# lijx10/SO-Net

Measured on AMD Instinct MI355X. Metric: point-clouds/sec forward, ModelNet40 5k-pt 8x8 SOM, higher is better.
Workload: dtype f32 (operands split into fp16 pieces, 3 fp16 MFMAs per product, f32 accumulate; parity 1e-5)

## Files before the change

include/sonet_hip.h:

```cpp
#ifndef SONET_HIP_H
#define SONET_HIP_H

#include <stddef.h>
#include <stdint.h>

#ifdef __cplusplus
extern "C" {
#endif

typedef void *sonet_stream_t;

enum {
    SONET_OK = 0,
    SONET_ERR_INVALID_ARG = 1,
    SONET_ERR_UNSUPPORTED = 2,
    SONET_ERR_LAUNCH = 3,
    SONET_ERR_NO_DEVICE = 4
};

int sonet_abi_version(void);
const char *sonet_build_arch(void);
const char *sonet_last_error(void);
int sonet_check_device(void);
int sonet_diag_mfma_f16_rate(int random_operands, int iters, double *tflops_out, double *ghz_out, sonet_stream_t stream);
// ... 208 lines not shown
                                  int B, int C, int L, sonet_stream_t stream);
int sonet_node_add_affine_act_f32(float *t, const float *z, const int32_t *min_idx_i32, const float *scale,
                                  const float *shift, int relu, int B, int C, int L, int M, sonet_stream_t stream);

size_t sonet_pointmlp_stats_ws_size(int B, int Cout, int L);
int sonet_pointmlp_h3_stats_f32(const float *x1, int C1, const float *x2, int C2, const void *Wp3, const float *scale,
                                const float *shift, int relu, float *y, int B, int Cout, int L, void *stats_ws,
                                float *mean, float *var, sonet_stream_t stream);
int sonet_pointmlp_x3_stats_f32(const float *x1, int C1, const float *x2, int C2, const void *Wp3, const float *scale,
                                const float *shift, int relu, float *y, int B, int Cout, int L, void *stats_ws,
                                float *mean, float *var, sonet_stream_t stream);

int sonet_pointmlp_h3_nodeadd_f32(const float *x1, int C1, const float *x2, int C2, const void *Wp3, const float *scale,
                                  const float *shift, int relu, float *y, int B, int Cout, int L,
                                  const float *zadd, const int32_t *zidx, int ZM, sonet_stream_t stream);
int sonet_pointmlp_h3_nodeadd_stats_f32(const float *x1, int C1, const float *x2, int C2, const void *Wp3, const float *scale,
                                        const float *shift, int relu, float *y, int B, int Cout, int L,
                                        const float *zadd, const int32_t *zidx, int ZM, void *stats_ws,
                                        float *mean, float *var, sonet_stream_t stream);

size_t sonet_pointmlp_bf16_stats_ws_size(int B, int Cout, int L);
int sonet_pointmlp_bf16_stats(const uint16_t *x1, int C1, const uint16_t *x2, int C2, const void *Wp,
                              const float *scale, const float *shift, int relu, uint16_t *y,
                              int B, int Cout, int L, void *stats_ws, float *mean, float *var, sonet_stream_t stream);
int sonet_pointmlp_bf16_pool(const uint16_t *x1, int C1, const uint16_t *x2, int C2, const void *Wp,
                             const float *scale, const float *shift, int relu, const int32_t *ids, const int32_t *row_max,
                             int32_t *out_idx, float *out_val, int B, int Cout, int L, int M, sonet_stream_t stream);
int sonet_pointmlp_bf16_stats_xaff(const uint16_t *x1, int C1, const uint16_t *x2, int C2, const void *Wp,
                                   const float *scale, const float *shift, int relu, uint16_t *y,
                                   int B, int Cout, int L, void *stats_ws, float *mean, float *var,
                                   const float *xs1, const float *xh1, const float *xs2, const float *xh2, int xrelu,
                                   sonet_stream_t stream);
int sonet_pointmlp_bf16_pool_xaff(const uint16_t *x1, int C1, const uint16_t *x2, int C2, const void *Wp,
                                  const float *scale, const float *shift, int relu, const int32_t *ids, const int32_t *row_max,
                                  int32_t *out_idx, float *out_val, int B, int Cout, int L, int M,
                                  const float *xs1, const float *xh1, const float *xs2, const float *xh2, int xrelu,
                                  sonet_stream_t stream);

size_t sonet_pointmlp_h3_segpool_ws_size(int B, int Cout, int M);
int sonet_pointmlp_h3_segpool_f32(const float *x1, int C1, const float *x2, int C2, const void *Wp3, const float *scale,
                                  const float *shift, int relu, const int32_t *ids_sorted, const int32_t *pos0,
                                  const int32_t *row_max, int M, void *ws, int32_t *out_idx, float *out_val,
                                  int B, int Cout, int L, const float *xs1, const float *xh1, const float *xs2, const float *xh2,
                                  int xrelu, sonet_stream_t stream);
int sonet_pointmlp_h3_stats_xaff_f32(const float *x1, int C1, const float *x2, int C2, const void *Wp3, const float *scale,
                                     const float *shift, int relu, float *y, int B, int Cout, int L, void *stats_ws,
                                     float *mean, float *var, const float *xs1, const float *xh1, const float *xs2, const float *xh2,
                                     int xrelu, sonet_stream_t stream);

size_t sonet_wgrad_x3_ws_size(int B, int Cout, int Cin, int L);
int sonet_wgrad_x3_f32(const float *g, const float *x, float *dw, void *ws, int B, int Cout, int Cin, int L, sonet_stream_t stream);
int sonet_wgrad_x3_xaff_f32(const float *g, const float *x, float *dw, void *ws, int B, int Cout, int Cin, int L,
                            const float *xs, const float *xh, int xrelu, sonet_stream_t stream);
size_t sonet_wgrad_bf16_ws_size(int B, int Cout, int Cin, int L);
int sonet_wgrad_bf16(const uint16_t *g, const uint16_t *x, float *dw, void *ws, int B, int Cout, int Cin, int L, sonet_stream_t stream);
int sonet_wgrad_bf16_xaff(const uint16_t *g, const uint16_t *x, float *dw, void *ws, int B, int Cout, int Cin, int L,
                          const float *xs, const float *xh, int xrelu, sonet_stream_t stream);
int sonet_node_gather_lead_affine_act_f32(const float *z, const int32_t *gidx, const float *lead, const float *wl,
                                          const float *scale, const float *shift, int relu, float *out,
                                          int B, int C, int L, int M, int NL, sonet_stream_t stream);

int sonet_node_gather_lead_affine_act_bf16(const uint16_t *z, const int32_t *gidx, const float *lead, const float *wl,
                                           const float *scale, const float *shift, int relu, uint16_t *out,
                                           int B, int C, int L, int M, int NL, sonet_stream_t stream);

int sonet_linear_act_f32(const float *x, const float *W, const float *scale, const float *shift, int relu, float *y,
                         int B, int Cin, int Cout, sonet_stream_t stream);

size_t sonet_pooled_dgrad_ws_size(int B, int C, int M, int L);
int sonet_pooled_wgrad_f32(const float *g_pooled, const int32_t *pos, const float *x, int B, int C, int M, int Ci, int L,
                           float *gw_partial, sonet_stream_t stream);
int sonet_pooled_wgrad_xaff_f32(const float *g_pooled, const int32_t *pos, const float *x, int B, int C, int M, int Ci, int L,
                                float *gw_partial, const float *xs, const float *xh, int xrelu, sonet_stream_t stream);
int sonet_pooled_dgrad_f32(const float *g_pooled, const int32_t *pos, const float *W, int B, int C, int M, int C1, int C2,
                           int L, void *ws, float *gx1, float *gx2, sonet_stream_t stream);
int sonet_pooled_wgrad_xbf16(const float *g_pooled, const int32_t *pos, const uint16_t *x, int B, int C, int M, int Ci, int L,
                             float *gw_partial, sonet_stream_t stream);
int sonet_pooled_wgrad_xaff_xbf16(const float *g_pooled, const int32_t *pos, const uint16_t *x, int B, int C, int M, int Ci, int L,
                                  float *gw_partial, const float *xs, const float *xh, int xrelu, sonet_stream_t stream);
int sonet_pooled_dgrad_obf16(const float *g_pooled, const int32_t *pos, const float *W, int B, int C, int M, int C1, int C2,
                             int L, void *ws, uint16_t *gx1, uint16_t *gx2, sonet_stream_t stream);
int sonet_pooled_dgrad_mfma_bf16(const float *g_pooled, const int32_t *pos, const void *wt_pack, int B, int C, int M, int C1, int C2,
                                 int L, void *ws, uint16_t *gx1, uint16_t *gx2, sonet_stream_t stream);

int sonet_bn_fwd_coeffs_f32(const float *mean, const float *var, const float *gamma, const float *beta, float eps, int C,
                            float *invstd, float *scale, float *shift, sonet_stream_t stream);
int sonet_bn_running_update_f32(float *running_mean, float *running_var, const float *mean, const float *var,
                                float momentum, float unbias, int C, sonet_stream_t stream);
int sonet_bn_rider_set(const float *gamma, const float *beta, float eps, float momentum, float unbias,
                       float *running_mean, float *running_var, float *invstd, float *scale, float *shift);
int sonet_bn_bwd_coeffs_f32(const double *sums, const float *mean, const float *invstd, const float *gamma, double n, int C,
                            float *a, float *b, float *c0, float *g_gamma, float *g_beta, sonet_stream_t stream);
int sonet_chunk_mean_f32(const float *h, float *out, long long rows, int N, int k, sonet_stream_t stream);
int sonet_channel_affine_act_out_f32(const float *x, const float *scale, const float *shift, int relu, float *y,
                                     int B, int C, int L, sonet_stream_t stream);

int sonet_channel_stats_f32(const float *y, int B, int C, int L, double *stat_ws,
                            float *mean, float *var_biased, sonet_stream_t stream);
int sonet_channel_affine_act_f32(float *y, const float *scale, const float *shift, int relu,
                                 int B, int C, int L, sonet_stream_t stream);

int sonet_chamfer_nn_f32(const float *q, const float *db, int32_t *nn, int B, int Nq, int Nd,
                         sonet_stream_t stream);
size_t sonet_chamfer_loss_ws_size(int B, int M, int N);
int sonet_chamfer_loss_f32(const float *pred, const float *gt, int32_t *nn_pg , int32_t *nn_gp ,
                           float *elem_fwd , float *elem_bwd , double *sums, void *ws, int B, int M,
                           int N, sonet_stream_t stream);
int sonet_chamfer_grad_f32(const float *pred, const float *gt, const int32_t *nn_pg, const int32_t *nn_gp, const float *elem_fwd,
                           const float *elem_bwd, const float *gscale, float *dpred, int32_t *bad, int B, int M, int N,
                           sonet_stream_t stream);
size_t sonet_seg_metrics_ws_size(int B, int C, int N);
int sonet_seg_metrics_f32(const float *score, const int64_t *seg, const int64_t *label, const int32_t *part_offsets, int n_cat,
                          int32_t *pred_out , int32_t *correct, double *nll_sum, int32_t *inter, int32_t *pred_cnt,
                          int32_t *gt_cnt, double *iou, int32_t *bad, void *ws, int B, int C, int N, sonet_stream_t stream);
int sonet_retrieval_chunk_keys(void);
size_t sonet_retrieval_ws_size(int N, int D, int Q, int top);
int sonet_retrieval_lists_f32(const float *feat, const int64_t *label , const int64_t *ids ,
                              const int32_t *query , int n_label, int top, int64_t *nn_id, float *nn_dist,
                              int32_t *nn_pos , int32_t *count, int32_t *label_out , int32_t *bad,
                              void *ws, int N, int D, int Q, sonet_stream_t stream);
#define SONET_UPCONV_TILE_PIXELS 128
#define SONET_UPCONV_K_CHUNK 16
#define SONET_UPCONV_COUT_BLOCK 32
#define SONET_UPCONV_MAX_HW 64
size_t sonet_upconv3x3_pack_size(int Cin, int Cout);
int sonet_upconv3x3_pack_f32(const float *W, void *Wp, int Cin, int Cout, sonet_stream_t stream);
int sonet_upconv3x3_f32(const float *x, const void *Wp, const float *scale, const float *shift, int relu, float *y,
                        int B, int Cin, int Cout, int H, int W, uint32_t *range_log, sonet_stream_t stream);
size_t sonet_upconv3x3_dgrad_pack_size(int Cin, int Cout);
int sonet_upconv3x3_dgrad_pack_f32(const float *W, void *Wpt, int Cin, int Cout, sonet_stream_t stream);
int sonet_upconv3x3_dgrad_f32(const float *g, const void *Wpt, float *dx, int B, int Cin, int Cout, int H, int W, sonet_stream_t stream);
#define SONET_UPWGRAD_K_STEP 16
#define SONET_UPWGRAD_CIN_BLOCK 32
#define SONET_UPWGRAD_FLUSH_COLS 256
#define SONET_UPWGRAD_SLICE_COLS 512
#define SONET_UPWGRAD_MAX_SLICES 128
size_t sonet_upconv3x3_wgrad_ws_size(int B, int Cin, int Cout, int H, int W);
int sonet_upconv3x3_wgrad_f32(const float *g, const float *x, float *dw, void *ws, int B, int Cin, int Cout, int H, int W,
                              sonet_stream_t stream);
#ifdef SONET_VARIANTS
int sonet_pointmlp_h3_kmax_f32(const float *x1, int C1, const float *x2, int C2, const void *Wp3, const float *scale,
                               const float *shift, int relu, float *out, void *keys_ws, int B, int Cout, int L, int M,
                               sonet_stream_t stream);

size_t sonet_chamfer_nn2_ws_size(int B, int Na, int Nb);
int sonet_chamfer_nn2_f32(const float *a, const float *b, int32_t *nn_ab, int32_t *nn_ba, void *ws, int B, int Na, int Nb,
                          sonet_stream_t stream);

size_t sonet_pooled_dgrad_tail_ws_size(int B, int C2, int L);
int sonet_pooled_dgrad_tail_f32(const float *g_pooled, const int32_t *pos, const float *W, int B, int C, int M, int C1, int C2,
                                int L, void *ws, float *gx1, float *gx2, const float *col0, const int32_t *pos0,
                                const float *sraw, const float *ssc, const float *ssh, int srelu, void *tail_ws, double *sums,
                                sonet_stream_t stream);
#endif

int sonet_pointmlp_x3_pack_strided(const float *W, long long row_stride, long long col_stride, void *Wp3, int Cin, int Cout, int rows,
                                   sonet_stream_t stream);
int sonet_pointmlp_h3_pack_strided(const float *W, long long row_stride, long long col_stride, void *Wp3, int Cin, int Cout, int rows,
                                   sonet_stream_t stream);
int sonet_pack_multi(const void *table, int n_entries, int total_blocks, sonet_stream_t stream);
int sonet_pack_multi_kc(int flavour, int Cin);
int sonet_pointmlp_bf16_pack_strided(const float *W, long long row_stride, long long col_stride, void *Wp, int Cin, int Cout, int rows,
                                     sonet_stream_t stream);

int sonet_adam_chunk(void);
int sonet_adam_multi_f32(const void *tensors, const float *step_size, const float *bc2_sqrt, const int32_t *chunk_tensor,
                         const long long *chunk_off, const long long *sizes, int nchunks, float beta1, float beta2,
                         float one_minus_beta1, float one_minus_beta2, float eps, sonet_stream_t stream);

int sonet_fc_max_rows(void);
int sonet_fc_bn_act_fwd_f32(const float *x, const float *W, const float *bias, const float *gamma, const float *beta,
                            float *running_mean, float *running_var, float momentum, float eps, int relu, int B, int Cin, int Cout,
                            float *y, float *xhat, float *invstd, sonet_stream_t stream);
int sonet_fc_bn_act_bwd_f32(const float *gy, const float *y, const float *xhat, const float *invstd, const float *gamma, const float *x,
                            int relu, int B, int Cin, int Cout, float *dz, float *dW, float *dbias, float *dgamma, float *dbeta,
                            sonet_stream_t stream);
int sonet_fc_dx_f32(const float *dz, const float *W, int B, int Cin, int Cout, float *dx, sonet_stream_t stream);

#ifdef __cplusplus
}
#endif
#endif
```

so-net_amd/csrc/knn_layer.hip:

```cpp
#include "common.hpp"
#include "knn_h1.hpp"

namespace {

constexpr int KL_STAGE = 8;
constexpr int KL_MAXC = 512;
constexpr int KL_WRING = 4;

struct KnnLayerArgs {
    const int4 *rec;
    const uint4 *zp;
    const float *wl, *scale1, *shift1;
    const uint4 *Wp;
    const float *scale2, *shift2;
    char *yp;
    unsigned *rlog;
    long long Lm;
    int relu1, relu2, KC, NS, KCP, CT, Cout, GK, G, ngout, Lout;
    int abl;
};

struct KnnLayerLds {
    uint4 x[2][KL_STAGE][2][2][128];
    float coef[5][KL_MAXC];
    float aff[KL_MAXC / 32][2][2][16];
    unsigned wmax[4];
};
static_assert(sizeof(KnnLayerLds) <= 160 * 1024, "LDS of a CU");
static_assert(4 * 32 * GM_STRIDE * sizeof(float) <= sizeof(uint4) * 2 * KL_STAGE * 2 * 2 * 128, "the epilogue's staging fits the operand buffers");

template <int MT>
__global__ __launch_bounds__(256) void knn_layer2_gmax_kernel(const KnnLayerArgs a)
{
    __shared__ __attribute__((aligned(16))) KnnLayerLds lds;
    const int tid = (int)threadIdx.x;
    const int lane = tid & 63, wave = __builtin_amdgcn_readfirstlane(tid >> 6);
    const int j = lane & 31, h = lane >> 5;
    const int blk = (int)blockIdx.x;
    const int col = tid & 127, hh = __builtin_amdgcn_readfirstlane(tid >> 7);
    const int4 rcol = a.rec[(long long)blk * 128 + col];
    const KnnCol kcol = knn_col(rcol);
    const int KC = a.KC, Cin = KC * 16;

    for (int t = tid; t < KL_MAXC; t += 256) {
        const int c = (t >> 4) * 16 + p16_channel((t >> 3) & 1, t & 7);
#pragma unroll
        for (int kind = 0; kind < 5; ++kind) lds.coef[kind][t] = knn_h1_coef(kind, c < Cin, c, a.wl, a.scale1, a.shift1);
    }
    for (int o = tid; o < a.Cout; o += 256) {
        const int rr = o & 31;
        float *t = &lds.aff[o >> 5][(rr >> 2) & 1][0][(rr & 3) | ((rr >> 3) << 2)];
        t[0] = a.scale2[o] * (32.f / 1024.f);
        t[16] = a.shift2[o] * 32.f;
    }

    RangeAcc xr = {0, 0u};
    const float lo1 = a.relu1 ? 0.f : -65504.f;
    const uint4 *zbase = a.zp + (long long)hh * a.Lm + (kcol.ok ? rcol.x : 0);

    uint4 Zh[2], Zm[2];
    unsigned hv4[4], mv4[4];
    f32x2_t creg[2][5];
    auto load_coef = [&](f32x2_t (&c)[5], int kc, int u) {
        const int ci = (kc < KC ? kc : KC - 1) * 16 + hh * 8 + 2 * u;
#pragma unroll
        for (int kind = 0; kind < 5; ++kind) c[kind] = *reinterpret_cast<const f32x2_t *>(&lds.coef[kind][ci]);
    };
    auto gather = [&](int slot, int kc) {
        kc = kc < KC ? kc : KC - 1;
        const uint4 *zq = zbase + (long long)kc * 4 * a.Lm;
#ifdef SONET_VARIANTS
        if (a.abl & 2) zq = a.zp + (long long)hh * a.Lm;
#endif
        Zh[slot] = zq[0];
        Zm[slot] = zq[2 * a.Lm];
    };
    auto build_unit = [&](int slot, const f32x2_t (&c)[5], int kc, int buf, int q, int u) {
        const bool in = kc < KC, live = kcol.ok && in;
        const float *const cf[5] = {reinterpret_cast<const float *>(&c[0]), reinterpret_cast<const float *>(&c[1]), reinterpret_cast<const float *>(&c[2]),
                                    reinterpret_cast<const float *>(&c[3]), reinterpret_cast<const float *>(&c[4])};
        KnnCol kk = kcol;
        kk.valid = kcol.valid && in;
        const unsigned zh = u == 0 ? Zh[slot].x : u == 1 ? Zh[slot].y : u == 2 ? Zh[slot].z : Zh[slot].w;
        const unsigned zm = u == 0 ? Zm[slot].x : u == 1 ? Zm[slot].y : u == 2 ? Zm[slot].z : Zm[slot].w;
        knn_h1_pair<false>(live ? zh : 0u, live ? zm : 0u, cf, kk, lo1, xr, hv4[u], mv4[u]);
        if (u == 3) {
            lds.x[buf][q][0][hh][col] = make_uint4(hv4[0], hv4[1], hv4[2], hv4[3]);
            lds.x[buf][q][1][hh][col] = make_uint4(mv4[0], mv4[1], mv4[2], mv4[3]);
        }
    };

    const int NS = a.NS, KCT = NS * KL_STAGE;
    const uint4 *wbase = a.Wp + ((size_t)(wave * MT) * a.KCP * 2) * 64 + lane;
    uint4 Wr[KL_WRING][2];
    auto load_w = [&](int kc0, int t) {
        int kc = kc0 + t / MT;
        kc = kc < KCT ? kc : KCT - 1;
        const uint4 *wq = wbase + ((size_t)(t % MT) * a.KCP + kc) * 128;
#ifdef SONET_VARIANTS
        if (a.abl & 1) wq = wbase;
#endif
        Wr[t % KL_WRING][0] = wq[0];
        Wr[t % KL_WRING][1] = wq[64];
    };

    f32x16 acc[MT][4];
#pragma unroll
    for (int mt = 0; mt < MT; ++mt)
#pragma unroll
        for (int c = 0; c < 4; ++c)
#pragma unroll
            for (int r = 0; r < 16; ++r) acc[mt][c][r] = 0.f;

    f16x8 Bf[2][2][4];
    auto read_b = [&](int set, int buf, int q) {
#pragma unroll
        for (int c = 0; c < 4; ++c) {
            Bf[set][0][c] = __builtin_bit_cast(f16x8, lds.x[buf][q][0][h][32 * c + j]);
            Bf[set][1][c] = __builtin_bit_cast(f16x8, lds.x[buf][q][1][h][32 * c + j]);
        }
    };

#pragma unroll
    for (int t = 0; t < KL_WRING - 1; ++t) load_w(0, t);
    {
        uint4 Ph[KL_STAGE], Pm[KL_STAGE];
#pragma unroll
        for (int q = 0; q < KL_STAGE; ++q) {
            gather(0, q);
            Ph[q] = Zh[0];
            Pm[q] = Zm[0];
        }
        __syncthreads();
#pragma unroll
        for (int q = 0; q < KL_STAGE; ++q) {
            Zh[0] = Ph[q];
            Zm[0] = Pm[q];
            f32x2_t c4[4][5];
#pragma unroll
            for (int u = 0; u < 4; ++u) load_coef(c4[u], q, u);
#pragma unroll
            for (int u = 0; u < 4; ++u) build_unit(0, c4[u], q, 0, q, u);
        }
    }
    if (NS > 1) load_coef(creg[0], KL_STAGE, 0);

    auto stage = [&](int s, auto build_next) {
        constexpr bool BUILD = decltype(build_next)::value;
        const int buf = s & 1, kc0 = s * KL_STAGE, kn = kc0 + KL_STAGE;
        __syncthreads();
        read_b(0, buf, 0);
        if constexpr (BUILD) gather(0, kn);
#pragma unroll
        for (int q = 0; q < KL_STAGE; ++q) {
#pragma unroll
            for (int mt = 0; mt < MT; ++mt) {
                const int t = q * MT + mt;
                load_w(kc0, t + KL_WRING - 1);
                if (mt == 0 && q + 1 < KL_STAGE) {
                    read_b((q + 1) & 1, buf, q + 1);
                    if constexpr (BUILD) gather((q + 1) & 1, kn + q + 1);
                }
                const f16x8 wh = __builtin_bit_cast(f16x8, Wr[t % KL_WRING][0]), wm = __builtin_bit_cast(f16x8, Wr[t % KL_WRING][1]);
#pragma unroll
                for (int term = 0; term < 3; ++term)
#pragma unroll
                    for (int c = 0; c < 4; ++c)
                        acc[mt][c] = __builtin_amdgcn_mfma_f32_32x32x16_f16(term == 0 ? wm : wh, Bf[q & 1][term == 1 ? 1 : 0][c], acc[mt][c], 0, 0, 0);
#pragma unroll
                for (int u = 0; u < 4; ++u)
                    if (BUILD && u * MT / 4 == mt) {
                        const int n = q * 4 + u;
                        load_coef(creg[(n + 1) & 1], kn + (n + 1) / 4, (n + 1) % 4);
                        build_unit(q & 1, creg[n & 1], kn + q, buf ^ 1, q, u);
                    }
#define KL_GAP2 __builtin_amdgcn_sched_group_barrier(0x008, 1, 0); __builtin_amdgcn_sched_group_barrier(0x002, 3, 0); \
                __builtin_amdgcn_sched_group_barrier(0x008, 1, 0); __builtin_amdgcn_sched_group_barrier(0x002, 4, 0);
                KL_GAP2 KL_GAP2 KL_GAP2 KL_GAP2 KL_GAP2 KL_GAP2
#undef KL_GAP2
                __builtin_amdgcn_sched_barrier(0);
            }
        }
    };
    for (int s = 0; s + 1 < NS; ++s) stage(s, bool_c<true>{});
    stage(NS - 1, bool_c<false>{});
    __syncthreads();

    float (*gm)[GM_STRIDE] = reinterpret_cast<float (*)[GM_STRIDE]>(reinterpret_cast<char *>(&lds.x[0][0][0][0][0]) + (size_t)wave * (32 * GM_STRIDE * 4));
    RangeAcc yr = {0, 0u};
    const float relu_thr = a.relu2 ? 0.f : -__builtin_inff();
    const float split_lo = a.relu2 ? 0.f : -2047.f;
    int tid2 = tid;
    asm volatile("" : "+v"(tid2));
    const int je = tid2 & 31, he = (tid2 >> 5) & 1;
    const int p = tid2 & 3, g = (tid2 & 63) >> 2;
    const long long n_out = (long long)blk * a.G + g;
    const bool node = g < a.G && n_out < a.ngout;
    const float *rbase = &gm[2 * (p & 1) + 8 * (p >> 1)][(g < a.G ? g : 0) * a.GK];
#pragma unroll
    for (int mt = 0; mt < MT; ++mt) {
        const int ct = wave * MT + mt;
        float sc16[16], sh16[16];
        {
            const float4 *t4 = reinterpret_cast<const float4 *>(&lds.aff[ct][he][0][0]);
#pragma unroll
            for (int u = 0; u < 4; ++u) {
                const float4 s4 = t4[u], h4 = t4[4 + u];
                sc16[4 * u] = s4.x; sc16[4 * u + 1] = s4.y; sc16[4 * u + 2] = s4.z; sc16[4 * u + 3] = s4.w;
                sh16[4 * u] = h4.x; sh16[4 * u + 1] = h4.y; sh16[4 * u + 2] = h4.z; sh16[4 * u + 3] = h4.w;
            }
        }
#pragma unroll
        for (int c = 0; c < 4; ++c)
#pragma unroll
            for (int r = 0; r < 16; ++r) {
                const float v = __fmaf_rn(acc[mt][c][r], sc16[r], sh16[r]);
                gm[(r & 3) + 8 * (r >> 2) + 4 * he][32 * c + je] = v < relu_thr ? 0.f : v;
            }
        __builtin_amdgcn_fence(__ATOMIC_RELEASE, "wavefront");
        __builtin_amdgcn_wave_barrier();
        __builtin_amdgcn_fence(__ATOMIC_ACQUIRE, "wavefront");
        float m0[4], m1[4];
#pragma unroll
        for (int qh = 0; qh < 4; ++qh) {
            const float *r0 = rbase + (16 * (qh >> 1) + 4 * (qh & 1)) * GM_STRIDE;
            m0[qh] = r0[0];
            m1[qh] = r0[GM_STRIDE];
        }
        for (int k = 1; k < a.GK; ++k) {
#pragma unroll
            for (int qh = 0; qh < 4; ++qh) {
                const float *r0 = rbase + (16 * (qh >> 1) + 4 * (qh & 1)) * GM_STRIDE;
                m0[qh] = nan_max(m0[qh], r0[k]);
                m1[qh] = nan_max(m1[qh], r0[GM_STRIDE + k]);
            }
        }
        if (node) {
#pragma unroll
            for (int qh = 0; qh < 4; ++qh) {
                const int qq = qh >> 1, h2 = qh & 1;
                gmax_p16_store(m0[qh], m1[qh], split_lo, yr, a.yp, ct * 2 + qq, h2, p, (size_t)a.Lout, (size_t)n_out);
            }
        }
        __builtin_amdgcn_fence(__ATOMIC_RELEASE, "wavefront");
        __builtin_amdgcn_wave_barrier();
        __builtin_amdgcn_fence(__ATOMIC_ACQUIRE, "wavefront");
    }

    if (a.rlog != nullptr) {
        const unsigned b1 = range_x32_out(wave_umax(range_act_bits(xr, a.relu1)));
        const unsigned b2 = range_x32_out(wave_umax(range_act_bits(yr, a.relu2)));
        if ((tid2 & 63) == 0) lds.wmax[wave] = b1 > b2 ? b1 : b2;
        __syncthreads();
        if (tid2 == 0) {
            const unsigned m01 = lds.wmax[0] > lds.wmax[1] ? lds.wmax[0] : lds.wmax[1], m23 = lds.wmax[2] > lds.wmax[3] ? lds.wmax[2] : lds.wmax[3];
            const unsigned mx = m01 > m23 ? m01 : m23;
            if (mx > __atomic_load_n(a.rlog + 2, __ATOMIC_RELAXED)) atomicMax(a.rlog + 2, mx);
            if (blk == 0) atomicMax(a.rlog + 1, reinterpret_cast<const unsigned *>(a.Wp + (size_t)a.CT * a.KCP * 128)[0]);
        }
    }
}

}

extern "C" int sonet_knn_layer2_gmax_p16(const void *rec, const void *z_p16, const float *wl, const float *scale1, const float *shift1, int relu1,
                                         int B, int M, int K, int Cin, const void *Wp, const float *scale2, const float *shift2, int relu2,
                                         int Cout, int GK, int G, int ngout, int Lout, void *yp, sonet_stream_t stream)
{
    const char *what = "sonet_knn_layer2_gmax_p16";
    SONET_REQUIRE(rec && z_p16 && wl && scale1 && shift1 && Wp && scale2 && shift2 && yp, "%s: NULL pointer", what);
    SONET_REQUIRE(B > 0 && M > 0 && Cin > 0 && Cout > 0 && K >= 1 && K <= 128, "%s: bad size B=%d M=%d Cin=%d Cout=%d K=%d", what, B, M, Cin, Cout, K);
    SONET_REQUIRE(GK == K && G == knn_stage_groups(K) && (long long)ngout == (long long)B * M, "%s: the grouping of the K-level layout is GK=%d G=%d ngout=%d", what,
                  K, knn_stage_groups(K), B * M);
    SONET_REQUIRE(Lout >= ngout, "%s: Lout=%d (the planes' column count) below ngout=%d", what, Lout, ngout);
    if (Cout % 128 != 0 || Cout > KL_MAXC) return sonet::fail(SONET_ERR_UNSUPPORTED, "%s: Cout=%d must be a multiple of 128, at most %d", what, Cout, KL_MAXC);
    if (Cin % 16 != 0 || Cin > KL_MAXC) return sonet::fail(SONET_ERR_UNSUPPORTED, "%s: Cin=%d must be a multiple of 16, at most %d", what, Cin, KL_MAXC);
    if (G * GK > 128) return sonet::fail(SONET_ERR_UNSUPPORTED, "%s: G GK = %d columns exceed a block", what, G * GK);
    const long long Lp = (long long)sonet_knn_stage_columns(B, M, K), Lm = (long long)sonet_node_stage_columns(B, M);
    const long long nblk = Lp / 128;
    const int KC = Cin / 16, NS = sonet::ceil_div(KC, KL_STAGE), KCP = NS * KL_STAGE, CT = Cout / 32;
    if (nblk > 0x7FFFFFFFll || (double)KC * 64.0 * (double)Lm >= 2.0e9 || (double)(Cout / 16) * 64.0 * (double)Lout >= 2.0e9 || (double)CT * KCP * 2048.0 >= 2.0e9)
        return sonet::fail(SONET_ERR_UNSUPPORTED, "%s: a panel exceeds 2 GiB", what);
    KnnLayerArgs a;
    a.rec = reinterpret_cast<const int4 *>(rec); a.zp = reinterpret_cast<const uint4 *>(z_p16); a.wl = wl; a.scale1 = scale1; a.shift1 = shift1;
    a.Wp = reinterpret_cast<const uint4 *>(Wp); a.scale2 = scale2; a.shift2 = shift2; a.yp = static_cast<char *>(yp); a.rlog = sonet::range_log();
    a.Lm = Lm; a.relu1 = relu1; a.relu2 = relu2; a.KC = KC; a.NS = NS; a.KCP = KCP; a.CT = CT; a.Cout = Cout; a.GK = GK; a.G = G; a.ngout = ngout; a.Lout = Lout;
    a.abl = 0;
#ifdef SONET_VARIANTS
    sonet::knob_int("SONET_KL_ABL", &a.abl);
#endif
    with_int_c<1, 2, 3, 4>(Cout / 128, [&](auto mt) {
        hipLaunchKernelGGL((knn_layer2_gmax_kernel<decltype(mt)::value>), dim3((unsigned)nblk), dim3(256), 0, sonet::as_stream(stream), a);
    });
    return sonet::launched(what);
}
```

so-net_amd/sonet_hip/_lib.py:

```python
import ctypes
import os

import torch

_HERE = os.path.dirname(os.path.abspath(__file__))
LIB_PATH = os.path.join(os.path.dirname(_HERE), "lib", "libsonet_hip.so")
VARIANTS_PATH = os.path.join(os.path.dirname(_HERE), "lib", "libsonet_hip_variants.so")
if os.environ.get("SONET_HIP_LIB"):
    LIB_PATH = os.environ["SONET_HIP_LIB"]

_vp = ctypes.c_void_p
_i = ctypes.c_int

SIGNATURES = {
    "sonet_abi_version": [],
    "sonet_build_arch": [],
    "sonet_last_error": [],
    "sonet_check_device": [],
    "sonet_range_log_set": [_vp],
    "sonet_pooled_wgrad_f32": [_vp, _vp, _vp, _i, _i, _i, _i, _i, _vp, _vp],
    "sonet_bn_running_update_f32": [_vp, _vp, _vp, _vp, ctypes.c_float, ctypes.c_float, _i, _vp],
    "sonet_knn_prepare_f32": [_vp, _vp, _i, _i, _i, _i, _vp, _vp, _vp, _vp],
    "sonet_pointmlp_h3_gather_f32": [_vp, _i, _i, _vp, _vp, _i, _vp, _vp, _vp, _i, _vp, _i, _i, _i, _vp],
    "sonet_planes_max_f32": [_vp, _vp, ctypes.c_longlong, _i, _i, _vp],
# ... 36 lines not shown
    "sonet_pointmlp_bf16_pack": [_vp, _vp, _i, _i, _vp],
    "sonet_pointmlp_bf16": [_vp, _i, _vp, _i, _vp, _vp, _vp, _i, _vp, _i, _i, _i, _vp],
    "sonet_pointmlp_bf16_acc": [_vp, _i, _vp, _i, _vp, _vp, _vp, _i, _vp, _vp, _i, _i, _i, _vp],
    "sonet_pointmlp_bf16_bnb": [_vp, _vp, _i, _vp, _vp, _vp, _vp, _vp, _vp, _vp, _vp, _i, _vp, _vp, _vp, _i, _i, _i, _vp],
    "sonet_pointmlp_bf16_gather": [_vp, _i, _i, _vp, _vp, _i, _vp, _vp, _vp, _i, _vp, _i, _i, _i, _vp],
    "sonet_index_max_gather_bf16": [_vp, _vp, _vp, _vp, _vp, _i, _i, _i, _i, _vp],
    "sonet_index_max_gather_p16": [_vp, _vp, _vp, _vp, _vp, _i, _i, _i, _i, _vp],
    "sonet_node_gather_lead_affine_act_f32": [_vp, _vp, _vp, _vp, _vp, _vp, _i, _vp, _i, _i, _i, _i, _i, _vp],
    "sonet_node_gather_lead_affine_act_bf16": [_vp, _vp, _vp, _vp, _vp, _vp, _i, _vp, _i, _i, _i, _i, _i, _vp],
    "sonet_pointmlp_stats_ws_size": [_i, _i, _i],
    "sonet_pointmlp_h3_stats_f32": [_vp, _i, _vp, _i, _vp, _vp, _vp, _i, _vp, _i, _i, _i, _vp, _vp, _vp, _vp],
    "sonet_pointmlp_x3_stats_f32": [_vp, _i, _vp, _i, _vp, _vp, _vp, _i, _vp, _i, _i, _i, _vp, _vp, _vp, _vp],
    "sonet_pointmlp_bf16_stats_ws_size": [_i, _i, _i],
    "sonet_pointmlp_bf16_stats": [_vp, _i, _vp, _i, _vp, _vp, _vp, _i, _vp, _i, _i, _i, _vp, _vp, _vp, _vp],
    "sonet_pointmlp_bf16_stats_xaff": [_vp, _i, _vp, _i, _vp, _vp, _vp, _i, _vp, _i, _i, _i, _vp, _vp, _vp, _vp, _vp, _vp, _vp, _i, _vp],
    "sonet_pointmlp_h3_nodeadd_f32": [_vp, _i, _vp, _i, _vp, _vp, _vp, _i, _vp, _i, _i, _i, _vp, _vp, _i, _vp],
    "sonet_pointmlp_h3_nodeadd_stats_f32": [_vp, _i, _vp, _i, _vp, _vp, _vp, _i, _vp, _i, _i, _i, _vp, _vp, _i, _vp, _vp, _vp, _vp],
    "sonet_wgrad_x3_ws_size": [_i, _i, _i, _i],
    "sonet_wgrad_x3_f32": [_vp, _vp, _vp, _vp, _i, _i, _i, _i, _vp],
    "sonet_wgrad_bf16_ws_size": [_i, _i, _i, _i],
    "sonet_wgrad_bf16": [_vp, _vp, _vp, _vp, _i, _i, _i, _i, _vp],
    "sonet_wgrad_bf16_xaff": [_vp, _vp, _vp, _vp, _i, _i, _i, _i, _vp, _vp, _i, _vp],
    "sonet_pointmlp_x3_pack_size": [_i, _i],
    "sonet_pointmlp_x3_pack": [_vp, _vp, _i, _i, _vp],
    "sonet_pointmlp_x3_f32": [_vp, _i, _vp, _i, _vp, _vp, _vp, _i, _vp, _i, _i, _i, _vp],
    "sonet_pointmlp_h3_pack": [_vp, _vp, _i, _i, _vp],
    "sonet_pointmlp_h3_f32": [_vp, _i, _vp, _i, _vp, _vp, _vp, _i, _vp, _i, _i, _i, _vp],
    "sonet_lastdim_argmax_f32": [_vp, _vp, _vp, ctypes.c_longlong, _i, _vp],
    "sonet_lastdim_argmax_bf16": [_vp, _vp, _vp, ctypes.c_longlong, _i, _vp],
    "sonet_lastdim_max_bwd_f32": [_vp, _vp, _vp, ctypes.c_longlong, _i, _vp],
    "sonet_lastdim_max_bwd_bf16": [_vp, _vp, _vp, ctypes.c_longlong, _i, _vp],
    "sonet_knn_gather_bwd_ws_size": [_i, _i, _i],
    "sonet_knn_gather_bwd_f32": [_vp, _vp, _vp, _vp, _i, _i, _i, _i, _vp],
    "sonet_knn_gather_bwd_bf16": [_vp, _vp, _vp, _vp, _i, _i, _i, _i, _vp],
    "sonet_node_gather_bwd_ws_size": [_i, _i, _i],
    "sonet_node_gather_bwd_f32": [_vp, _vp, _vp, _vp, _i, _i, _i, _i, _vp],
    "sonet_node_gather_bwd_bf16": [_vp, _vp, _vp, _vp, _i, _i, _i, _i, _vp],
    "sonet_pointwise_bwd_apply_nodesum_ws_size": [_i, _i, _i],
    "sonet_pointwise_bwd_apply_nodesum_tile": [],
    "sonet_pointwise_bwd_apply_nodesum_f32": [_vp, _vp, _vp, _vp, _i, _vp, _vp, _vp, _vp, _i, _vp, _vp, _vp, _i, _i, _i, _vp],
    "sonet_p16_size": [_i, _i, _i],
    "sonet_p16_from_f32": [_vp, _vp, _i, _i, _i, _vp, _vp, _i, _vp],
    "sonet_p16_to_f32": [_vp, _vp, _i, _i, _i, _vp],
    "sonet_pointmlp_h3p_pack_size": [_i, _i],
    "sonet_pointmlp_h3p_pack": [_vp, _vp, _i, _i, _vp],
    "sonet_pointmlp_h3p_stats_ws_size": [_i, _i, _i],
    "sonet_pointmlp_h3p": [_vp, _i, _i, _vp, _vp, _i, _vp, _vp, _vp, _i, _vp, _vp, _i, _i, _i, _vp, _vp, _i, _vp, _vp, _vp, _vp],
    "sonet_pointresnet_bf16_pack_size": [],
    "sonet_pointresnet_bf16_pack": [_vp, _vp, _vp, _vp, _i, _vp, _vp],
    "sonet_pointresnet_bf16": [_vp, _i, _vp, _vp, _vp, _i, _i, _vp],
    "sonet_pointresnet_bf16_pool_ws_size": [_i, _i, _i],
    "sonet_pointresnet_bf16_pool": [_vp, _i, _vp, _vp, _vp, _vp, _vp, _vp, _vp, _vp, _i, _i, _i, _vp],
    "sonet_pointresnet_pack_size": [],
    "sonet_pointresnet_pack": [_vp, _vp, _vp, _vp, _i, _vp, _vp],
    "sonet_pointresnet_fused_f32": [_vp, _i, _vp, _vp, _vp, _i, _i, _vp],
    "sonet_pointresnet_fused_p16_f32": [_vp, _i, _vp, _vp, _vp, _vp, _i, _i, _vp],
    "sonet_pointresnet_pool_ws_size": [_i, _i, _i],
    "sonet_pointresnet_fused_pool_f32": [_vp, _i, _vp, _vp, _vp, _vp, _vp, _vp, _vp, _vp, _i, _i, _i, _vp],
    "sonet_pointresnet_fused_pool_p16_f32": [_vp, _i, _vp, _vp, _vp, _vp, _vp, _vp, _vp, _vp, _vp, _i, _i, _i, _vp],
    "sonet_knn_stage_columns": [_i, _i, _i],
    "sonet_knn_stage_prepare_f32": [_vp, _vp, _i, _i, _i, _i, _i, _vp, _vp, _vp, _vp],
    "sonet_knn_stage_input_p16": [_vp, _vp, _vp, _vp, _vp, _i, _i, _i, _i, _i, _vp, _vp],
    "sonet_pointmlp_h3p_gmax": [_vp, _i, _vp, _i, _vp, _vp, _vp, _i, _i, _i, _i, _i, _i, _i, _vp, _vp, _vp],
    "sonet_knn_layer2_gmax_p16": [_vp, _vp, _vp, _vp, _vp, _i, _i, _i, _i, _i, _vp, _vp, _vp, _i, _i, _i, _i, _i, _i, _vp, _vp],
    "sonet_node_stage_columns": [_i, _i],
    "sonet_p16_flat_to_bcm_f32": [_vp, _vp, _i, _i, _i, _vp],
    "sonet_som_sort_group_f32": [_vp, _vp, _vp, _vp, _vp, _i, _i, _i, _i, _vp, _vp, _vp, _vp, _vp, _vp, _vp, _vp],
    "sonet_pointwise_bwd_stats_f32": [_vp, _vp, _vp, _vp, _i, _i, _i, _i, _vp, _vp],
    "sonet_pointwise_bwd_apply_f32": [_vp, _vp, _vp, _vp, _i, _vp, _vp, _vp, _vp, _i, _i, _i, _vp],
    "sonet_node_add_affine_act_f32": [_vp, _vp, _vp, _vp, _vp, _i, _i, _i, _i, _i, _vp],
    "sonet_linear_act_f32": [_vp, _vp, _vp, _vp, _i, _vp, _i, _i, _i, _vp],
    "sonet_pooled_dgrad_ws_size": [_i, _i, _i, _i],
    "sonet_pooled_wgrad_xbf16": [_vp, _vp, _vp, _i, _i, _i, _i, _i, _vp, _vp],
    "sonet_pooled_wgrad_xaff_xbf16": [_vp, _vp, _vp, _i, _i, _i, _i, _i, _vp, _vp, _vp, _i, _vp],
    "sonet_pooled_dgrad_obf16": [_vp, _vp, _vp, _i, _i, _i, _i, _i, _i, _vp, _vp, _vp, _vp],
    "sonet_pooled_dgrad_f32": [_vp, _vp, _vp, _i, _i, _i, _i, _i, _i, _vp, _vp, _vp, _vp],
    "sonet_pooled_dgrad_mfma_bf16": [_vp, _vp, _vp, _i, _i, _i, _i, _i, _i, _vp, _vp, _vp, _vp],
    "sonet_bn_fwd_coeffs_f32": [_vp, _vp, _vp, _vp, ctypes.c_float, _i, _vp, _vp, _vp, _vp],
    "sonet_bn_bwd_coeffs_f32": [_vp, _vp, _vp, _vp, ctypes.c_double, _i, _vp, _vp, _vp, _vp, _vp, _vp],
    "sonet_channel_affine_act_out_f32": [_vp, _vp, _vp, _i, _vp, _i, _i, _i, _vp],
    "sonet_chunk_mean_f32": [_vp, _vp, ctypes.c_longlong, _i, _i, _vp],
    "sonet_pointmlp_x3_pack_strided": [_vp, ctypes.c_longlong, ctypes.c_longlong, _vp, _i, _i, _i, _vp],
    "sonet_pointmlp_h3_pack_strided": [_vp, ctypes.c_longlong, ctypes.c_longlong, _vp, _i, _i, _i, _vp],
    "sonet_pointmlp_bf16_pack_strided": [_vp, ctypes.c_longlong, ctypes.c_longlong, _vp, _i, _i, _i, _vp],
    "sonet_adam_chunk": [],
    "sonet_fc_max_rows": [],
    "sonet_fc_bn_act_fwd_f32": [_vp, _vp, _vp, _vp, _vp, _vp, _vp, ctypes.c_float, ctypes.c_float, _i, _i, _i, _i, _vp, _vp, _vp, _vp],
    "sonet_fc_bn_act_bwd_f32": [_vp, _vp, _vp, _vp, _vp, _vp, _i, _i, _i, _i, _vp, _vp, _vp, _vp, _vp, _vp],
    "sonet_fc_dx_f32": [_vp, _vp, _i, _i, _i, _vp, _vp],
    "sonet_adam_multi_f32": [_vp, _vp, _vp, _vp, _vp, _vp, _i, ctypes.c_float, ctypes.c_float, ctypes.c_float, ctypes.c_float, ctypes.c_float, _vp],
    "sonet_channel_stats_f32": [_vp, _i, _i, _i, _vp, _vp, _vp, _vp],
    "sonet_channel_stats_bf16": [_vp, _i, _i, _i, _vp, _vp, _vp, _vp],
    "sonet_channel_affine_act_out_bf16": [_vp, _vp, _vp, _i, _vp, _i, _i, _i, _vp],
    "sonet_pointwise_bwd_stats_bf16": [_vp, _vp, _vp, _vp, _i, _i, _i, _i, _vp, _vp],
    "sonet_pointwise_bwd_apply_bf16": [_vp, _vp, _vp, _vp, _i, _vp, _vp, _vp, _vp, _i, _i, _i, _vp],
    "sonet_channel_affine_act_f32": [_vp, _vp, _vp, _i, _i, _i, _i, _vp],
    "sonet_chamfer_nn_f32": [_vp, _vp, _vp, _i, _i, _i, _vp],
    "sonet_chamfer_loss_ws_size": [_i, _i, _i],
    "sonet_chamfer_loss_f32": [_vp, _vp, _vp, _vp, _vp, _vp, _vp, _vp, _i, _i, _i, _vp],
    "sonet_chamfer_grad_f32": [_vp, _vp, _vp, _vp, _vp, _vp, _vp, _vp, _vp, _i, _i, _i, _vp],
    "sonet_upconv3x3_pack_size": [_i, _i],
    "sonet_upconv3x3_pack_f32": [_vp, _vp, _i, _i, _vp],
    "sonet_upconv3x3_f32": [_vp, _vp, _vp, _vp, _i, _vp, _i, _i, _i, _i, _i, _vp, _vp],
    "sonet_upconv3x3_dgrad_pack_size": [_i, _i],
    "sonet_upconv3x3_dgrad_pack_f32": [_vp, _vp, _i, _i, _vp],
    "sonet_upconv3x3_dgrad_f32": [_vp, _vp, _vp, _i, _i, _i, _i, _i, _vp],
    "sonet_upconv3x3_wgrad_ws_size": [_i, _i, _i, _i, _i],
    "sonet_upconv3x3_wgrad_f32": [_vp, _vp, _vp, _vp, _i, _i, _i, _i, _i, _vp],
    "sonet_seg_metrics_ws_size": [_i, _i, _i],
    "sonet_seg_metrics_f32": [_vp, _vp, _vp, _vp, _i, _vp, _vp, _vp, _vp, _vp, _vp, _vp, _vp, _vp, _i, _i, _i, _vp],
    "sonet_retrieval_chunk_keys": [],
    "sonet_retrieval_ws_size": [_i, _i, _i, _i],
    "sonet_retrieval_lists_f32": [_vp, _vp, _vp, _vp, _i, _i, _vp, _vp, _vp, _vp, _vp, _vp, _vp, _i, _i, _i, _vp],
}
_RESTYPES = {
    "sonet_build_arch": ctypes.c_char_p,
    "sonet_last_error": ctypes.c_char_p,
    "sonet_pointmlp_pack_size": ctypes.c_size_t,
    "sonet_pointmlp_stats_ws_size": ctypes.c_size_t,
    "sonet_pointmlp_h3_segpool_ws_size": ctypes.c_size_t,
    "sonet_pointmlp_bf16_stats_ws_size": ctypes.c_size_t,
    "sonet_wgrad_x3_ws_size": ctypes.c_size_t,
    "sonet_wgrad_bf16_ws_size": ctypes.c_size_t,
    "sonet_pointmlp_x3_pack_size": ctypes.c_size_t,
    "sonet_p16_size": ctypes.c_size_t,
    "sonet_knn_stage_columns": ctypes.c_size_t,
    "sonet_node_stage_columns": ctypes.c_size_t,
    "sonet_knn_gather_bwd_ws_size": ctypes.c_size_t,
    "sonet_node_gather_bwd_ws_size": ctypes.c_size_t,
    "sonet_pointwise_bwd_apply_nodesum_ws_size": ctypes.c_size_t,
    "sonet_pointmlp_h3p_pack_size": ctypes.c_size_t,
    "sonet_pointmlp_h3p_stats_ws_size": ctypes.c_size_t,
    "sonet_pointmlp_bf16_pack_size": ctypes.c_size_t,
    "sonet_pointresnet_pack_size": ctypes.c_size_t,
    "sonet_pointresnet_bf16_pack_size": ctypes.c_size_t,
    "sonet_pointresnet_bf16_pool_ws_size": ctypes.c_size_t,
    "sonet_pointresnet_pool_ws_size": ctypes.c_size_t,
    "sonet_pooled_dgrad_ws_size": ctypes.c_size_t,
    "sonet_pooled_dgrad_tail_ws_size": ctypes.c_size_t,
    "sonet_som_assign_sort_ws_size": ctypes.c_size_t,
    "sonet_chamfer_nn2_ws_size": ctypes.c_size_t,
    "sonet_chamfer_loss_ws_size": ctypes.c_size_t,
    "sonet_upconv3x3_pack_size": ctypes.c_size_t,
    "sonet_upconv3x3_dgrad_pack_size": ctypes.c_size_t,
    "sonet_upconv3x3_wgrad_ws_size": ctypes.c_size_t,
    "sonet_seg_metrics_ws_size": ctypes.c_size_t,
    "sonet_retrieval_ws_size": ctypes.c_size_t,
}

VARIANT_SIGNATURES = {
    "sonet_chamfer_nn2_ws_size": [_i, _i, _i],
    "sonet_chamfer_nn2_f32": [_vp, _vp, _vp, _vp, _vp, _i, _i, _i, _vp],
    "sonet_pointmlp_h3_kmax_f32": [_vp, _i, _vp, _i, _vp, _vp, _vp, _i, _vp, _vp, _i, _i, _i, _i, _vp],
    "sonet_pooled_dgrad_tail_ws_size": [_i, _i, _i],
    "sonet_pooled_dgrad_tail_f32": [_vp, _vp, _vp, _i, _i, _i, _i, _i, _i, _vp, _vp, _vp, _vp, _vp, _vp, _vp, _vp, _i, _vp, _vp, _vp],
}

_lib = None


class SonetHipError(RuntimeError):
    pass


def load():
    global _lib
    if _lib is not None:
        return _lib
    if not os.path.exists(LIB_PATH):
        raise SonetHipError(
            "libsonet_hip.so is not built (%s).  Build it with `make -C so-net_amd/csrc` or "
            "`python -c 'import __graft_entry__ as g; g.build()'`.  There is no CPU fallback." % LIB_PATH)
    try:
        lib = ctypes.CDLL(LIB_PATH)
    except OSError as e:
        raise SonetHipError("cannot load %s: %s" % (LIB_PATH, e))
    for name, args in SIGNATURES.items():
        fn = getattr(lib, name)
        fn.argtypes = args
        fn.restype = _RESTYPES.get(name, ctypes.c_int)
    for name, args in VARIANT_SIGNATURES.items():
        fn = getattr(lib, name, None)
        if fn is not None:
            fn.argtypes = args
            fn.restype = _RESTYPES.get(name, ctypes.c_int)
    _lib = lib
    return lib


def last_error():
    return load().sonet_last_error().decode("utf-8", "replace")


def check(status, what=""):
    if status != 0:
        raise SonetHipError("%s failed (status %d): %s" % (what or "libsonet_hip", status, last_error()))


_device_ok = {}


def require_device(device):
    if device.index in _device_ok:
        return
    if device.type != "cuda" and torch.cuda.is_available():
        raise SonetHipError("sonet_hip needs its tensors on an MI355X (gfx950) GPU, got one on %s; there is no CPU fallback" % device)
    if not torch.cuda.is_available():
        raise SonetHipError("sonet_hip needs an MI355X (gfx950) GPU; torch.cuda.is_available() is False "
                            "and there is no CPU fallback")
    idx = device.index if device.index is not None else torch.cuda.current_device()
    ok = _device_ok.get(idx)
    if ok is None:
        with torch.cuda.device(idx):
            check(load().sonet_check_device(), "sonet_check_device")
        _device_ok[idx] = True


def stream_ptr():
    return ctypes.c_void_p(torch._C._cuda_getCurrentRawStream(torch._C._cuda_getDevice()))


class on_device:
    __slots__ = ("idx", "prev")

    def __init__(self, dev):
        self.idx = dev.index if dev.index is not None else -1

    def __enter__(self):
        self.prev = torch.cuda._exchange_device(self.idx)

    def __exit__(self, *exc):
        torch.cuda._maybe_exchange_device(self.prev)
        return False


def ptr(t):
    return ctypes.c_void_p(t.data_ptr()) if t is not None else None
```

Baseline: 75020.

## Restructure knn layer2 epilogue with double-buffered swizzled staging and overlapped table loads

The epilogue now stages each output tile into one of two per-wave LDS areas as XOR-swizzled float4 rows and reduces columns with vectorized reads. Staging of tile mt+1 is overlapped with the max-reduction of tile mt, and the reduction is specialised at compile time for GK of 9 and 16. The coefficient and affine tables are loaded into registers up front and written to LDS only after the first operand gathers are issued, hiding their global-load latency. A profiling instrumentation path, compiled only in the variants build, is also added; the extra register use of the hoisted tables and wider staging could lower occupancy.

After: 75270, median of 6. Within noise of the previous version (+0.3%).

```diff
diff --git a/include/sonet_hip.h b/include/sonet_hip.h
--- a/include/sonet_hip.h
+++ b/include/sonet_hip.h
@@ -384,6 +384,8 @@
                                 int L, void *ws, float *gx1, float *gx2, const float *col0, const int32_t *pos0,
                                 const float *sraw, const float *ssc, const float *ssh, int srelu, void *tail_ws, double *sums,
                                 sonet_stream_t stream);
+
+int sonet_knn_layer2_prof_read(long long *host, int n);
 #endif
 
 int sonet_pointmlp_x3_pack_strided(const float *W, long long row_stride, long long col_stride, void *Wp3, int Cin, int Cout, int rows,
diff --git a/so-net_amd/csrc/knn_layer.hip b/so-net_amd/csrc/knn_layer.hip
--- a/so-net_amd/csrc/knn_layer.hip
+++ b/so-net_amd/csrc/knn_layer.hip
@@ -27,11 +27,27 @@
     unsigned wmax[4];
 };
 static_assert(sizeof(KnnLayerLds) <= 160 * 1024, "LDS of a CU");
-static_assert(4 * 32 * GM_STRIDE * sizeof(float) <= sizeof(uint4) * 2 * KL_STAGE * 2 * 2 * 128, "the epilogue's staging fits the operand buffers");
-
-template <int MT>
+constexpr int KL_EPI_AREA = 128 * 32 * 4;
+static_assert(4 * 2 * KL_EPI_AREA <= sizeof(uint4) * 2 * KL_STAGE * 2 * 2 * 128, "the epilogue's staging (two areas per wave) fits the operand buffers");
+
+#ifdef SONET_VARIANTS
+constexpr int KL_PROF_N = 16, KL_PROF_BLOCKS = 1024;
+__device__ long long g_kl_prof[KL_PROF_BLOCKS * 4 * KL_PROF_N];
+#define KL_PROF_DECL long long prof_rt0_ = 0, prof_t_ = 0;                                                                                       \
+    if constexpr (PROF) { prof_rt0_ = (long long)__builtin_amdgcn_s_memrealtime(); prof_t_ = __builtin_readcyclecounter(); }
+#define KL_PROF_PUT(i, v) if ((threadIdx.x & 63) == 0 && blockIdx.x < KL_PROF_BLOCKS) g_kl_prof[(blockIdx.x * 4 + (threadIdx.x >> 6)) * KL_PROF_N + (i)] = (v);
+#define KL_PROF_MARK(i) if constexpr (PROF) { const long long n_ = __builtin_readcyclecounter(); KL_PROF_PUT(i, n_ - prof_t_) prof_t_ = n_; }
+#define KL_PROF_DUMP if constexpr (PROF) { KL_PROF_PUT(15, (long long)__builtin_amdgcn_s_memrealtime() - prof_rt0_) }
+#else
+#define KL_PROF_DECL
+#define KL_PROF_MARK(i)
+#define KL_PROF_DUMP
+#endif
+
+template <int MT, bool PROF>
 __global__ __launch_bounds__(256) void knn_layer2_gmax_kernel(const KnnLayerArgs a)
 {
+    KL_PROF_DECL
     __shared__ __attribute__((aligned(16))) KnnLayerLds lds;
     const int tid = (int)threadIdx.x;
     const int lane = tid & 63, wave = __builtin_amdgcn_readfirstlane(tid >> 6);
@@ -42,17 +58,29 @@
     const KnnCol kcol = knn_col(rcol);
     const int KC = a.KC, Cin = KC * 16;
 
-    for (int t = tid; t < KL_MAXC; t += 256) {
+    constexpr int KL_TABR = KL_MAXC / 256;
+    float cv[KL_TABR][5], av[KL_TABR][2];
+#pragma unroll
+    for (int i = 0; i < KL_TABR; ++i) {
+        const int t = tid + 256 * i;
         const int c = (t >> 4) * 16 + p16_channel((t >> 3) & 1, t & 7);
 #pragma unroll
-        for (int kind = 0; kind < 5; ++kind) lds.coef[kind][t] = knn_h1_coef(kind, c < Cin, c, a.wl, a.scale1, a.shift1);
+        for (int kind = 0; kind < 5; ++kind) cv[i][kind] = knn_h1_coef(kind, true, c < Cin ? c : 0, a.wl, a.scale1, a.shift1);
+        av[i][0] = a.scale2[t < a.Cout ? t : 0];
+        av[i][1] = a.shift2[t < a.Cout ? t : 0];
     }
-    for (int o = tid; o < a.Cout; o += 256) {
-        const int rr = o & 31;
-        float *t = &lds.aff[o >> 5][(rr >> 2) & 1][0][(rr & 3) | ((rr >> 3) << 2)];
-        t[0] = a.scale2[o] * (32.f / 1024.f);
-        t[16] = a.shift2[o] * 32.f;
-    }
+    auto store_tables = [&]() {
+#pragma unroll
+        for (int i = 0; i < KL_TABR; ++i) {
+            const int t = tid + 256 * i, c = (t >> 4) * 16 + p16_channel((t >> 3) & 1, t & 7);
+#pragma unroll
+            for (int kind = 0; kind < 5; ++kind) lds.coef[kind][t] = c < Cin ? cv[i][kind] : 0.f;
+            const int rr = t & 31;
+            float *q = &lds.aff[t >> 5][(rr >> 2) & 1][0][(rr & 3) | ((rr >> 3) << 2)];
+            q[0] = av[i][0] * (32.f / 1024.f);
+            q[16] = av[i][1] * 32.f;
+        }
+    };
 
     RangeAcc xr = {0, 0u};
     const float lo1 = a.relu1 ? 0.f : -65504.f;
@@ -131,7 +159,9 @@
             Ph[q] = Zh[0];
             Pm[q] = Zm[0];
         }
+        store_tables();
         __syncthreads();
+        KL_PROF_MARK(0)
 #pragma unroll
         for (int q = 0; q < KL_STAGE; ++q) {
             Zh[0] = Ph[q];
@@ -143,6 +173,7 @@
             for (int u = 0; u < 4; ++u) build_unit(0, c4[u], q, 0, q, u);
         }
     }
+    KL_PROF_MARK(1)
     if (NS > 1) load_coef(creg[0], KL_STAGE, 0);
 
     auto stage = [&](int s, auto build_next) {
@@ -181,24 +212,25 @@
                 __builtin_amdgcn_sched_barrier(0);
             }
         }
+        KL_PROF_MARK(2 + s)
     };
     for (int s = 0; s + 1 < NS; ++s) stage(s, bool_c<true>{});
     stage(NS - 1, bool_c<false>{});
     __syncthreads();
 
-    float (*gm)[GM_STRIDE] = reinterpret_cast<float (*)[GM_STRIDE]>(reinterpret_cast<char *>(&lds.x[0][0][0][0][0]) + (size_t)wave * (32 * GM_STRIDE * 4));
+    char *const garea = reinterpret_cast<char *>(&lds.x[0][0][0][0][0]) + (size_t)wave * (2 * KL_EPI_AREA);
     RangeAcc yr = {0, 0u};
     const float relu_thr = a.relu2 ? 0.f : -__builtin_inff();
     const float split_lo = a.relu2 ? 0.f : -2047.f;
     int tid2 = tid;
     asm volatile("" : "+v"(tid2));
     const int je = tid2 & 31, he = (tid2 >> 5) & 1;
-    const int p = tid2 & 3, g = (tid2 & 63) >> 2;
+    const int h2 = tid2 & 1, pp = (tid2 >> 1) & 1, g = (tid2 & 63) >> 2;
     const long long n_out = (long long)blk * a.G + g;
     const bool node = g < a.G && n_out < a.ngout;
-    const float *rbase = &gm[2 * (p & 1) + 8 * (p >> 1)][(g < a.G ? g : 0) * a.GK];
-#pragma unroll
-    for (int mt = 0; mt < MT; ++mt) {
+    const int c0 = (g < a.G ? g : 0) * a.GK;
+#define KL_WAVE_SYNC __builtin_amdgcn_fence(__ATOMIC_RELEASE, "wavefront"); __builtin_amdgcn_wave_barrier(); __builtin_amdgcn_fence(__ATOMIC_ACQUIRE, "wavefront");
+    auto stage_tile = [&](int mt) {
         const int ct = wave * MT + mt;
         float sc16[16], sh16[16];
         {
@@ -210,41 +242,72 @@
                 sh16[4 * u] = h4.x; sh16[4 * u + 1] = h4.y; sh16[4 * u + 2] = h4.z; sh16[4 * u + 3] = h4.w;
             }
         }
+        char *const wr = garea + (mt & 1) * KL_EPI_AREA + je * 128;
 #pragma unroll
         for (int c = 0; c < 4; ++c)
 #pragma unroll
-            for (int r = 0; r < 16; ++r) {
-                const float v = __fmaf_rn(acc[mt][c][r], sc16[r], sh16[r]);
-                gm[(r & 3) + 8 * (r >> 2) + 4 * he][32 * c + je] = v < relu_thr ? 0.f : v;
-            }
-        __builtin_amdgcn_fence(__ATOMIC_RELEASE, "wavefront");
-        __builtin_amdgcn_wave_barrier();
-        __builtin_amdgcn_fence(__ATOMIC_ACQUIRE, "wavefront");
-        float m0[4], m1[4];
-#pragma unroll
-        for (int qh = 0; qh < 4; ++qh) {
-            const float *r0 = rbase + (16 * (qh >> 1) + 4 * (qh & 1)) * GM_STRIDE;
-            m0[qh] = r0[0];
-            m1[qh] = r0[GM_STRIDE];
-        }
-        for (int k = 1; k < a.GK; ++k) {
-#pragma unroll
-            for (int qh = 0; qh < 4; ++qh) {
-                const float *r0 = rbase + (16 * (qh >> 1) + 4 * (qh & 1)) * GM_STRIDE;
-                m0[qh] = nan_max(m0[qh], r0[k]);
-                m1[qh] = nan_max(m1[qh], r0[GM_STRIDE + k]);
-            }
+            for (int u = 0; u < 4; ++u) {
+                float v[4];
+#pragma unroll
+                for (int i = 0; i < 4; ++i) {
+                    const float f = __fmaf_rn(acc[mt][c][4 * u + i], sc16[4 * u + i], sh16[4 * u + i]);
+                    v[i] = f < relu_thr ? 0.f : f;
+                }
+                *reinterpret_cast<float4 *>(wr + c * (32 * 128) + (((2 * u + he) ^ ((je >> 1) & 7)) << 4)) = make_float4(v[0], v[1], v[2], v[3]);
+            }
+    };
+    auto reduce_tile = [&](int mt, auto gkc) {
+        constexpr int GKC = decltype(gkc)::value;
+        const int ct = wave * MT + mt;
+        const char *const rd = garea + (mt & 1) * KL_EPI_AREA;
+        float m[2][4];
+        auto column = [&](int k) {
+            const int cc = c0 + k, key = (cc >> 1) & 7;
+#pragma unroll
+            for (int qq = 0; qq < 2; ++qq) {
+                const float4 v = *reinterpret_cast<const float4 *>(rd + cc * 128 + (((4 * qq + 2 * pp + h2) ^ key) << 4));
+                if (k == 0) {
+                    m[qq][0] = v.x; m[qq][1] = v.y; m[qq][2] = v.z; m[qq][3] = v.w;
+                } else {
+                    m[qq][0] = nan_max(m[qq][0], v.x); m[qq][1] = nan_max(m[qq][1], v.y);
+                    m[qq][2] = nan_max(m[qq][2], v.z); m[qq][3] = nan_max(m[qq][3], v.w);
+                }
+            }
+        };
+        column(0);
+        if constexpr (GKC != 0) {
+#pragma unroll
+            for (int k = 1; k < GKC; ++k) column(k);
+        } else {
+            for (int k = 1; k < a.GK; ++k) column(k);
         }
         if (node) {
 #pragma unroll
-            for (int qh = 0; qh < 4; ++qh) {
-                const int qq = qh >> 1, h2 = qh & 1;
-                gmax_p16_store(m0[qh], m1[qh], split_lo, yr, a.yp, ct * 2 + qq, h2, p, (size_t)a.Lout, (size_t)n_out);
-            }
-        }
-        __builtin_amdgcn_fence(__ATOMIC_RELEASE, "wavefront");
-        __builtin_amdgcn_wave_barrier();
-        __builtin_amdgcn_fence(__ATOMIC_ACQUIRE, "wavefront");
+            for (int qq = 0; qq < 2; ++qq)
+#pragma unroll
+                for (int e = 0; e < 2; ++e)
+                    gmax_p16_store(m[qq][2 * e], m[qq][2 * e + 1], split_lo, yr, a.yp, ct * 2 + qq, h2, 2 * pp + e, (size_t)a.Lout, (size_t)n_out);
+        }
+    };
+    auto epilogue = [&](auto gkc) {
+        stage_tile(0);
+        KL_WAVE_SYNC
+#pragma unroll
+        for (int mt = 0; mt < MT; ++mt) {
+            if (mt + 1 < MT) {
+                stage_tile(mt + 1);
+                KL_WAVE_SYNC
+            }
+            reduce_tile(mt, gkc);
+            KL_WAVE_SYNC
+            KL_PROF_MARK(7 + mt)
+        }
+    };
+#undef KL_WAVE_SYNC
+    switch (a.GK) {
+    case 9: epilogue(int_c<9>{}); break;
+    case 16: epilogue(int_c<16>{}); break;
+    default: epilogue(int_c<0>{}); break;
     }
 
     if (a.rlog != nullptr) {
@@ -259,6 +322,8 @@
             if (blk == 0) atomicMax(a.rlog + 1, reinterpret_cast<const unsigned *>(a.Wp + (size_t)a.CT * a.KCP * 128)[0]);
         }
     }
+    KL_PROF_MARK(11)
+    KL_PROF_DUMP
 }
 
 }
@@ -289,8 +354,27 @@
 #ifdef SONET_VARIANTS
     sonet::knob_int("SONET_KL_ABL", &a.abl);
 #endif
+    int prof = 0;
+#ifdef SONET_VARIANTS
+    sonet::knob_int("SONET_KL_PROF", &prof);
+#endif
     with_int_c<1, 2, 3, 4>(Cout / 128, [&](auto mt) {
-        hipLaunchKernelGGL((knn_layer2_gmax_kernel<decltype(mt)::value>), dim3((unsigned)nblk), dim3(256), 0, sonet::as_stream(stream), a);
+        constexpr int MT = decltype(mt)::value;
+#ifdef SONET_VARIANTS
+        if (prof) {
+            hipLaunchKernelGGL((knn_layer2_gmax_kernel<MT, true>), dim3((unsigned)nblk), dim3(256), 0, sonet::as_stream(stream), a);
+            return;
+        }
+#endif
+        hipLaunchKernelGGL((knn_layer2_gmax_kernel<MT, false>), dim3((unsigned)nblk), dim3(256), 0, sonet::as_stream(stream), a);
     });
+    (void)prof;
     return sonet::launched(what);
 }
+
+#ifdef SONET_VARIANTS
+extern "C" int sonet_knn_layer2_prof_read(long long *host, int n)
+{
+    return hipMemcpyFromSymbol(host, HIP_SYMBOL(g_kl_prof), sizeof(long long) * (size_t)n, 0, hipMemcpyDeviceToHost) == hipSuccess ? 0 : 1;
+}
+#endif
diff --git a/so-net_amd/sonet_hip/_lib.py b/so-net_amd/sonet_hip/_lib.py
--- a/so-net_amd/sonet_hip/_lib.py
+++ b/so-net_amd/sonet_hip/_lib.py
@@ -212,6 +212,7 @@
     "sonet_chamfer_nn2_ws_size": [_i, _i, _i],
     "sonet_chamfer_nn2_f32": [_vp, _vp, _vp, _vp, _vp, _i, _i, _i, _vp],
     "sonet_pointmlp_h3_kmax_f32": [_vp, _i, _vp, _i, _vp, _vp, _vp, _i, _vp, _vp, _i, _i, _i, _i, _vp],
+    "sonet_knn_layer2_prof_read": [_vp, _i],
     "sonet_pooled_dgrad_tail_ws_size": [_i, _i, _i],
     "sonet_pooled_dgrad_tail_f32": [_vp, _vp, _vp, _i, _i, _i, _i, _i, _i, _vp, _vp, _vp, _vp, _vp, _vp, _vp, _vp, _i, _vp, _vp, _vp],
 }
```
